# JanSpindler/NRC-HPM-Renderer

Hardware: AMD Instinct MI355X
Metric: Msamples/s + ms/frame at 1080p, 256^3 cloud (NRC path) (higher is better)
Workload: dtype f16 (fp16 MFMA operands, fp32 accumulate; fp32 integrator)

## Files before the change

include/nrc_hpm.h:

```cpp
#ifndef NRC_HPM_H
#define NRC_HPM_H
#include <stddef.h>
#include <stdint.h>

#ifdef __cplusplus
extern "C" {
#endif

#define NRC_OK 0
#define NRC_ERR_INVALID (-1)
#define NRC_ERR_HIP (-2)
#define NRC_ERR_STATE (-3)
#define NRC_ERR_COMM (-4)

const char* nrc_last_error(void);
const char* nrc_version(void);

typedef struct nrc_config {
    char loss_fn[32];
    char optimizer[32];
    float learning_rate;
    float ema_decay;
    uint32_t pos_id;
    uint32_t dir_id;
// ... 130 lines not shown
int nrc_renderer_set_schedule(nrc_renderer_t* r, const nrc_schedule* schedule);
int nrc_renderer_get_schedule(nrc_renderer_t* r, nrc_schedule* current, int* tuning_done);
const char* nrc_renderer_schedule_source(nrc_renderer_t* r);
const char* nrc_renderer_schedule_key(nrc_renderer_t* r);
int nrc_schedule_cache_load(const char* path, int* n_entries);
int nrc_schedule_cache_save(const char* path, int* n_entries);
int nrc_schedule_cache_clear(void);
int nrc_renderer_set_cost_order(nrc_renderer_t* r, int on);
size_t nrc_renderer_tile_order(nrc_renderer_t* r, uint32_t* host_out, size_t capacity);
int nrc_renderer_set_hot_tiles(nrc_renderer_t* r, int on);
int nrc_renderer_hot_tiles(nrc_renderer_t* r, uint32_t* host_out9);
int nrc_renderer_set_full_vertex_images(nrc_renderer_t* r, int on);
size_t nrc_renderer_vertex_image_bytes(nrc_renderer_t* r);
int nrc_renderer_set_stage_events(nrc_renderer_t* r, int on);
int nrc_renderer_count_fetches(nrc_renderer_t* r, int enable, unsigned long long* out);
int nrc_renderer_train_grid(nrc_renderer_t* r, uint32_t out5[5]);

typedef struct nrc_mc_renderer nrc_mc_renderer_t;

int nrc_mc_renderer_create(uint32_t width, uint32_t height, uint32_t path_length, int blend, const nrc_camera* camera,
                           const nrc_scene* scene, const nrc_tile* tile, void* stream, nrc_mc_renderer_t** out);
int nrc_mc_renderer_render(nrc_mc_renderer_t* r);
int nrc_mc_renderer_set_camera(nrc_mc_renderer_t* r, const nrc_camera* camera);
int nrc_mc_renderer_set_blend(nrc_mc_renderer_t* r, int blend);
int nrc_mc_renderer_set_empty_skip(nrc_mc_renderer_t* r, int on);
int nrc_mc_renderer_set_cost_order(nrc_mc_renderer_t* r, int on);
int nrc_mc_renderer_is_blending(nrc_mc_renderer_t* r);
int nrc_mc_renderer_set_scene_params(nrc_mc_renderer_t* r, const nrc_scene* scene);
int nrc_mc_renderer_set_frame_random(nrc_mc_renderer_t* r, const float random4[4]);
const float* nrc_mc_renderer_framebuffer(nrc_mc_renderer_t* r);
int nrc_mc_renderer_export_exr(nrc_mc_renderer_t* r, const char* path);
float nrc_mc_renderer_frame_time_ms(nrc_mc_renderer_t* r);
int nrc_mc_renderer_count_fetches(nrc_mc_renderer_t* r, int enable, unsigned long long* out);
int nrc_mc_renderer_destroy(nrc_mc_renderer_t* r);

int nrc_compare_images(const float* d_ref_rgba, const float* d_own_rgba, uint32_t w, uint32_t h, void* stream,
                       float result5[5]);

int nrc_compare_images_sharded(nrc_cache_t* comm, const float* d_ref_local_rgba, const float* d_own_local_rgba, uint32_t n_local_pixels,
                               void* stream, float result5[5]);

// ... 13 lines not shown
```

nrc-hpm-renderer_amd/api.py:

```python
import ctypes as C
import os

import numpy as np

_HERE = os.path.dirname(os.path.abspath(__file__))
LIB_PATH = os.environ.get("NRC_HPM_LIB") or os.path.join(_HERE, "lib", "libnrc_hpm.so")

NRC_FIX_Q1_TRAIN_Y_DIST = 1
NRC_FIX_Q2_TRAIN_RAY_LEN = 2


class NrcConfig(C.Structure):
    _fields_ = [
        ("loss_fn", C.c_char * 32), ("optimizer", C.c_char * 32),
        ("learning_rate", C.c_float), ("ema_decay", C.c_float),
        ("pos_id", C.c_uint32), ("dir_id", C.c_uint32), ("nn_width", C.c_uint32), ("nn_depth", C.c_uint32),
        ("log2_infer_batch_size", C.c_uint32), ("log2_train_batch_size", C.c_uint32), ("train_batch_count", C.c_uint32),
        ("scene_id", C.c_uint32), ("train_ring_buf_size", C.c_float), ("train_spp", C.c_uint32),
        ("primary_ray_length", C.c_uint32), ("primary_ray_prob", C.c_float), ("train_ray_length", C.c_uint32),
        ("seed", C.c_uint32), ("compat_fix", C.c_uint32), ("hashgrid_log2_size", C.c_uint32),
    ]


class NrcScene(C.Structure):
# ... 29 lines not shown
    "nrc_renderer_set_cost_order", "nrc_renderer_set_schedule", "nrc_renderer_get_schedule", "nrc_renderer_schedule_source", "nrc_renderer_schedule_key",
    "nrc_schedule_cache_load", "nrc_schedule_cache_save", "nrc_schedule_cache_clear", "nrc_renderer_tile_order", "nrc_mc_renderer_set_cost_order", "nrc_renderer_set_hot_tiles", "nrc_renderer_hot_tiles",
    "nrc_cache_get_infer_batch_count", "nrc_cache_get_train_batch_count", "nrc_cache_get_infer_batch_size",
    "nrc_cache_get_train_batch_size", "nrc_cache_infer", "nrc_cache_backward", "nrc_cache_optimizer_step",
    "nrc_cache_grad_ptr", "nrc_cache_param_count", "nrc_cache_loss_ptr", "nrc_cache_set_loss_norm_factor",
    "nrc_comm_unique_id", "nrc_cache_comm_init", "nrc_cache_comm_sparse", "nrc_cache_grid_list_capacity",
    "nrc_cache_set_exchange_dtype", "nrc_cache_get_exchange_dtype",
    "nrc_cache_grid_grad_pack", "nrc_cache_grid_grad_apply",
    "nrc_cache_set_stream", "nrc_cache_set_grad_hook", "nrc_cache_get_params", "nrc_cache_set_params",
    "nrc_cache_get_step", "nrc_cache_set_step", "nrc_cache_param_count_tcnn", "nrc_cache_get_params_tcnn", "nrc_cache_set_params_tcnn",
    "nrc_cache_save_checkpoint", "nrc_cache_load_checkpoint", "nrc_cache_comm_status", "nrc_cache_set_comm_timeout_ms",
    "nrc_renderer_create", "nrc_renderer_render", "nrc_renderer_render_frames", "nrc_renderer_set_stage_events", "nrc_renderer_set_camera", "nrc_renderer_set_blend",
    "nrc_renderer_set_scene_params", "nrc_mc_renderer_set_scene_params",
    "nrc_renderer_set_show_nrc", "nrc_renderer_set_frame_random", "nrc_renderer_framebuffer", "nrc_renderer_framebuffer_on",
    "nrc_renderer_export_exr",
    "nrc_renderer_frame_time_ms", "nrc_renderer_stage_stats", "nrc_renderer_frame_timeline", "nrc_set_wave_priority_raise", "nrc_renderer_destroy", "nrc_renderer_buffer", "nrc_renderer_count_fetches",
    "nrc_renderer_train_grid",
    "nrc_mc_renderer_create", "nrc_mc_renderer_render", "nrc_mc_renderer_set_camera", "nrc_mc_renderer_set_blend",
    "nrc_mc_renderer_set_frame_random", "nrc_mc_renderer_framebuffer", "nrc_mc_renderer_export_exr",
    "nrc_mc_renderer_frame_time_ms", "nrc_mc_renderer_count_fetches", "nrc_mc_renderer_destroy",
    "nrc_compare_images", "nrc_test_math", "nrc_test_rng", "nrc_debug_check_guards", "nrc_image_create", "nrc_image_destroy",
]

_lib = None


def set_wave_priority_raise(on=True):
    _check(load_library().nrc_set_wave_priority_raise(C.c_int(int(bool(on)))))


def build_id():
# ... 581 lines not shown
            return _wrap_device(p, nbytes.value, torch.int32, (nbytes.value // 4,))
        inner = {"primary": 4, "info": 1, "origin": 4, "dir": 4, "infer_input": 5, "infer_output": 3,
                 "train_input": 5, "train_target": 3}[name]
        return _wrap_device(p, nbytes.value, torch.float32, (nbytes.value // (4 * inner), inner))

    def TrainGrid(self):
        o = (C.c_uint32 * 5)()
        _check(self.L.nrc_renderer_train_grid(self.h, o))
        return dict(tw=o[0], th=o[1], x_dist=o[2], y_dist=o[3], ring_size=o[4])

    def CountFetches(self, enable=True):
        v = C.c_ulonglong(0)
        _check(self.L.nrc_renderer_count_fetches(self.h, C.c_int(int(enable)), C.byref(v)))
        return v.value

    def Destroy(self):
        if self.h:
            _check(self.L.nrc_renderer_destroy(self.h))
            self.h = None

    def __del__(self):
        try:
            self.Destroy()
        except Exception:
            pass


class McHpmRenderer:

    def __init__(self, width, height, pathLength, blend, camera, scene, tile=None, stream=None):
# ... 39 lines not shown
        _check(self.L.nrc_mc_renderer_export_exr(self.h, filePath.encode()))

    def GetFrameTimeMS(self):
        return float(self.L.nrc_mc_renderer_frame_time_ms(self.h))

    def GetImage(self):
        import torch
        p = self.L.nrc_mc_renderer_framebuffer(self.h)
        return _wrap_device(p, self.width * self.height * 16, torch.float32, (self.height, self.width, 4))

    def CountFetches(self, enable=True):
        v = C.c_ulonglong(0)
        _check(self.L.nrc_mc_renderer_count_fetches(self.h, C.c_int(int(enable)), C.byref(v)))
        return v.value

    def Destroy(self):
        if self.h:
            _check(self.L.nrc_mc_renderer_destroy(self.h))
            self.h = None

    def __del__(self):
        try:
            self.Destroy()
        except Exception:
            pass


def comm_unique_id():
    buf = (C.c_char * 128)()
    _check(load_library().nrc_comm_unique_id(buf))
# ... 40 lines not shown
```

nrc-hpm-renderer_amd/csrc/nrc_api.hip:

```cpp
#include <algorithm>
#include <array>
#include <chrono>
#include <cmath>
#include <cstdio>
#include <cstdlib>
#include <cstring>
#include <fstream>
#include <map>
#include <memory>
#include <mutex>
#include <random>
#include <string>
#include <thread>
#include <unordered_map>
#include <vector>

#include <dlfcn.h>
#include <rccl/rccl.h>

#include "nrc_integrator.hpp"
#include "nrc_mlp.hpp"
#include "build_id.h"

namespace nrc {
// ... 697 lines not shown
            for (uint32_t y = 0; y < s.ny; y++) {
                const uint8_t* row = s.density + ((size_t)z * s.ny + y) * s.nx;
                const size_t base = ((size_t)(z >> sh) * gy + (y >> sh)) * gx;
                for (uint32_t x = 0; x < s.nx; x++)
                    if (row[x]) {
                        const size_t cidx = base + (x >> sh);
                        bits[cidx >> 5] |= 1u << (cidx & 31);
                    }
            }
        dev_alloc(&d_occ_bits, bits.size() * 4, "d_occ_bits");
        NRC_HIP(hipMemcpy(d_occ_bits, bits.data(), bits.size() * 4, hipMemcpyHostToDevice));
        d.occ_bits = (const uint32_t*)d_occ_bits;
        d.occ_shift = sh; d.occ_gx = gx; d.occ_gy = gy; d.occ_words = (uint32_t)bits.size();
    }

    void build_occupancy(const nrc_scene& s)
    {
        const uint32_t nx = s.nx, ny = s.ny, nz = s.nz;
        const uint32_t gx = (nx + 7) / 8, gy = (ny + 7) / 8, gz = (nz + 7) / 8;
        std::vector<uint8_t> occ((size_t)gx * gy * gz, 0);
        for (uint32_t z = 0; z < nz; z++)
            for (uint32_t y = 0; y < ny; y++) {
                const uint8_t* row = s.density + ((size_t)z * ny + y) * nx;
                const uint32_t cz0 = (z ? z - 1 : 0) >> 3, cz1 = std::min(z + 1, nz - 1) >> 3;
                const uint32_t cy0 = (y ? y - 1 : 0) >> 3, cy1 = std::min(y + 1, ny - 1) >> 3;
                for (uint32_t x = 0; x < nx; x++) {
                    if (row[x] == 0) continue;
                    const uint32_t cx0 = (x ? x - 1 : 0) >> 3, cx1 = std::min(x + 1, nx - 1) >> 3;
                    for (uint32_t cz = cz0; cz <= cz1; cz++)
                        for (uint32_t cy = cy0; cy <= cy1; cy++)
// ... 37 lines not shown
        d.fnx = (float)s.nx; d.fny = (float)s.ny; d.fnz = (float)s.nz;
        float size[3] = {s.size[0], s.size[1], s.size[2]};
        if (size[0] == 0.0f && size[1] == 0.0f && size[2] == 0.0f) {
            const float l = sqrtf((d.fnx * d.fnx + d.fny * d.fny) + d.fnz * d.fnz);
            size[0] = d.fnx / l * 107.5f; size[1] = d.fny / l * 107.5f; size[2] = d.fnz / l * 107.5f;
        }
        for (int k = 0; k < 3; k++) {
            d.size[k] = size[k];
            d.half_size[k] = size[k] * 0.5f;
            d.inv_size[k] = 1.0f / size[k];
        }
        const float tx = 2.0f * size[0], ty = 2.0f * size[1], tz = 2.0f * size[2];
        d.len2size = sqrtf(fmaf(tz, tz, fmaf(ty, ty, tx * tx)));
        build_occupancy(s);
        build_occupancy_bits(s);
        set_params(s);
        d.env = nullptr; d.env_w = d.env_h = 0;
        if (s.env && s.env_w && s.env_h) {
            const size_t eb = (size_t)s.env_w * s.env_h * 16;
            dev_alloc(&d_env, eb, "d_env");
            NRC_HIP(hipMemcpy(d_env, s.env, eb, hipMemcpyHostToDevice));
            d.env = (const float*)d_env; d.env_w = s.env_w; d.env_h = s.env_h;
        }
    }
    void set_params(const nrc_scene& s)
    {
        if (!(s.density_factor > 0.0f)) fail("scene density factor must be positive");
        d.density_factor = s.density_factor;
        d.inv_max_density = 1.0f / s.density_factor;
        d.g = s.g;
// ... 814 lines not shown
    {
        if (frame_index_ > 0)
            NRC_HIP(hipStreamWaitEvent(consumer, ev_comp_done_[(frame_index_ - 1) % (uint64_t)kGenSets], 0));
    }
    void release_frame(hipStream_t consumer)
    {
        if (!ev_consumer_) NRC_HIP(hipEventCreateWithFlags(&ev_consumer_, hipEventDisableTiming));
        NRC_HIP(hipEventRecord(ev_consumer_, consumer));
        consumer_pending_ = true;
    }
    bool is_blending() const { return blend_; }
    void set_full_vertex_images(bool on) { full_vertex_images_ = on; }
    size_t vertex_image_bytes() const { return (full_vertex_images_ ? (size_t)w_ * h_ : (size_t)tg_.tw * tg_.th) * 32; }
    const float* framebuffer_unordered() const { return (const float*)d_out_; }
    const TrainGrid& train_grid() const { return tg_; }
    hipStream_t stream() const { return stream_; }

private:
    void alloc(void** p, size_t bytes)
    {
        dev_alloc(p, bytes, "renderer buffer");
        NRC_HIP(hipMemset(*p, 0, bytes));
        allocs_.push_back(*p);
    }

    void calc_train_subset(uint32_t train_pixel_count)
    {
        const uint32_t sq = (uint32_t)std::sqrt((double)train_pixel_count);
        for (uint32_t factor = sq; factor >= 2; factor--) {
            if (train_pixel_count % factor == 0) {
// ... 326 lines not shown
        timed_ = true;
    }
    void set_cost_order(bool on) { cost_order_ = on; }
    void set_camera(const nrc_camera& c)
    {
        cam_ = to_dev(c);
        nrc_cam_ = c;
        mask_dirty_ = true;
        order_fresh_ = 2;
        blend_index_ = 1;
        NRC_HIP(hipMemsetAsync(d_out_, 0, (size_t)w_ * h_ * 16, stream_));
    }
    void set_scene_params(const nrc_scene& s) { scene_.set_params(s); mask_dirty_ = true; }
    void set_blend(bool b) { blend_ = b; blend_index_ = 1; }
    bool is_blending() const { return blend_; }
    void set_frame_random(const float* r) { std::memcpy(pinned_random_, r, 16); have_pinned_random_ = true; }
    void set_count_fetches(bool on) { count_fetches_ = on; NRC_HIP(hipMemsetAsync(d_fetch_, 0, 8, stream_)); }
    unsigned long long fetches()
    {
        unsigned long long v = 0;
        NRC_HIP(hipMemcpyAsync(&v, d_fetch_, 8, hipMemcpyDeviceToHost, stream_));
        NRC_HIP(hipStreamSynchronize(stream_));
        return v;
    }
    float frame_time_ms()
    {
        if (!timed_) return 0.0f;
        float ms = 0;
        NRC_HIP(hipEventSynchronize(ev_[1]));
        NRC_HIP(hipEventElapsedTime(&ms, ev_[0], ev_[1]));
// ... 548 lines not shown
    NRC_REQUIRE(cam); NRC_REQUIRE(scene); NRC_REQUIRE(out);
    return guarded([&] { *out = new nrc_mc_renderer(w, h, path_length, blend != 0, *cam, *scene, tile, (hipStream_t)stream); });
}
int nrc_mc_renderer_render(nrc_mc_renderer_t* r) { NRC_REQUIRE(r); return guarded([&] { r->impl.render(); }); }
int nrc_mc_renderer_set_camera(nrc_mc_renderer_t* r, const nrc_camera* c) { NRC_REQUIRE(r); NRC_REQUIRE(c); return guarded([&] { r->impl.set_camera(*c); }); }
int nrc_mc_renderer_set_blend(nrc_mc_renderer_t* r, int b) { NRC_REQUIRE(r); r->impl.set_blend(b != 0); return NRC_OK; }
int nrc_mc_renderer_set_frame_random(nrc_mc_renderer_t* r, const float* v) { NRC_REQUIRE(r); NRC_REQUIRE(v); r->impl.set_frame_random(v); return NRC_OK; }
const float* nrc_mc_renderer_framebuffer(nrc_mc_renderer_t* r) { return r ? r->impl.framebuffer() : nullptr; }
int nrc_mc_renderer_export_exr(nrc_mc_renderer_t* r, const char* path) { NRC_REQUIRE(r); NRC_REQUIRE(path); return guarded([&] { r->impl.export_exr(path); }); }
float nrc_mc_renderer_frame_time_ms(nrc_mc_renderer_t* r)
{
    float v = -1.0f;
    if (r) guarded([&] { v = r->impl.frame_time_ms(); });
    return v;
}
int nrc_mc_renderer_count_fetches(nrc_mc_renderer_t* r, int enable, unsigned long long* out)
{
    NRC_REQUIRE(r);
    return guarded([&] { if (out) *out = r->impl.fetches(); r->impl.set_count_fetches(enable != 0); });
}
int nrc_mc_renderer_destroy(nrc_mc_renderer_t* r)
{
    if (!r) return NRC_OK;
    return guarded([&] { delete r; });
}

int nrc_compare_images(const float* d_ref, const float* d_own, uint32_t w, uint32_t h, void* stream, float result5[5])
{
    NRC_REQUIRE(d_ref); NRC_REQUIRE(d_own); NRC_REQUIRE(result5);
    return guarded([&] {
// ... 97 lines not shown
```

nrc-hpm-renderer_amd/csrc/nrc_integrator.hip:

```cpp
#include "nrc_integrator.hpp"

#include <cstdlib>
#include <string>

#include "nrc_math.h"

#ifndef NRC_OCC_ALWAYS
#define NRC_OCC_ALWAYS 0
#endif
#ifndef NRC_CAMERA_WAVES_PER_SIMD
#define NRC_CAMERA_WAVES_PER_SIMD 5
#endif

namespace nrc {
namespace {

struct V3 {
    float x, y, z;
};
__device__ __forceinline__ V3 v3(float x, float y, float z) { return V3{x, y, z}; }
__device__ __forceinline__ V3 add(V3 a, V3 b) { return v3(a.x + b.x, a.y + b.y, a.z + b.z); }
__device__ __forceinline__ V3 sub(V3 a, V3 b) { return v3(a.x - b.x, a.y - b.y, a.z - b.z); }
__device__ __forceinline__ V3 mul(V3 a, float s) { return v3(a.x * s, a.y * s, a.z * s); }
__device__ __forceinline__ V3 neg(V3 a) { return v3(-a.x, -a.y, -a.z); }
// ... 84 lines not shown
        }                                                                                 \
    } while (0)
#define NRC_PROF_LIVE(which, mask)                                                           \
    do {                                                                                     \
        const int n_ = __popcll(mask);                                                       \
        if (n_ > 0 && (threadIdx.x & 63u) == 0u) {                                           \
            const int cls_ = n_ <= 1 ? 0 : n_ <= 2 ? 1 : n_ <= 4 ? 2 : n_ <= 8 ? 3 : n_ <= 16 ? 4 : n_ <= 32 ? 5 : 6; \
            atomicAdd(&g_live_hist[which][cls_], 1ull);                                      \
        }                                                                                    \
    } while (0)
#else
#define NRC_PROF(c, k) do { } while (0)
#define NRC_PROF_LIVE(which, mask) do { } while (0)
#endif

template <bool COUNT>
struct CtxT {
    const DevScene& sc;
    float rng;
    uint32_t fetches;
    __amdgpu_buffer_rsrc_t vol = __builtin_amdgcn_make_buffer_rsrc((void*)sc.density, 0, (int)(sc.nx * sc.ny * sc.nz), 0x00020000);
    const uint32_t* occ = nullptr;
#ifdef NRC_LOOP_PROFILE
    uint32_t useful[8] = {0, 0, 0, 0, 0, 0, 0, 0}, issued[8] = {0, 0, 0, 0, 0, 0, 0, 0};
    uint32_t fee_kind = 1;
#endif
#ifdef NRC_DIAG_CUT_TAIL2
    uint32_t cut2 = 0;
#endif
    __device__ __forceinline__ float rand(float max_val)
    {
        rng = random1(rng);
        return rng * max_val;
    }
    __device__ __forceinline__ void count(uint32_t n)
    {
        if constexpr (COUNT) fetches += n;
    }
};

__device__ __forceinline__ const uint32_t* load_occupancy(const DevScene& sc, uint32_t* s_occ)
{
    fill_log_table();
    if (sc.occ_bits == nullptr) return nullptr;
    for (uint32_t i = threadIdx.x; i < sc.occ_words; i += blockDim.x) s_occ[i] = sc.occ_bits[i];
    __syncthreads();
    return s_occ;
}
__device__ __forceinline__ const uint32_t* load_occupancy_per_wave(const DevScene& sc, uint32_t* s_occ)
{
    fill_log_table();
    if (sc.occ_bits == nullptr) return nullptr;
    const uint4* src = reinterpret_cast<const uint4*>(sc.occ_bits);
    uint4* dst = reinterpret_cast<uint4*>(s_occ);
    for (uint32_t i = threadIdx.x & 63u; i < (sc.occ_words >> 2); i += 64u) dst[i] = src[i];
// ... 81 lines not shown
    const uint32_t ix = (uint32_t)fx, iy = (uint32_t)fy, iz = (uint32_t)fz;
    uint32_t idx = index24(iz, s.ny, iy, s.nx, ix);
    idx = inb ? idx : 0u;
    const uint8_t t = s.density[idx];
    const float d = s.density_factor * ((float)t * (1.0f / 255.0f));
    return inb ? d : 0.0f;
}

struct Addr2 {
    uint32_t i0, i1;
};
struct Fetch2 {
    uint32_t b0, b1;
};
template <class C>
__device__ __forceinline__ Addr2 fetch2_addr(const C& c, V3 dir, V3 start, float t1, float t2, bool first, bool second)
{
    const DevScene& s = c.sc;
    const f2 t = f2{t1, t2};
    const f2 px = fma2(splat(dir.x), t, splat(start.x));
    const f2 py = fma2(splat(dir.y), t, splat(start.y));
    const f2 pz = fma2(splat(dir.z), t, splat(start.z));
    const f2 u = fma2(px, splat(s.inv_size[0]), splat(0.5f));
    const f2 v = fma2(py, splat(s.inv_size[1]), splat(0.5f));
    const f2 w = fma2(pz, splat(s.inv_size[2]), splat(0.5f));
    const f2 fx = u * splat(s.fnx), fy = v * splat(s.fny), fz = w * splat(s.fnz);
    bool in0 = (max(max(nrc_f2u(u.x), nrc_f2u(v.x)), nrc_f2u(w.x)) < 0x3f800000u) & first;
    bool in1 = (max(max(nrc_f2u(u.y), nrc_f2u(v.y)), nrc_f2u(w.y)) < 0x3f800000u) & second;
    const uint32_t x0 = (uint32_t)fx.x, y0 = (uint32_t)fy.x, z0 = (uint32_t)fz.x;
    const uint32_t x1 = (uint32_t)fx.y, y1 = (uint32_t)fy.y, z1 = (uint32_t)fz.y;
    const uint32_t idx0 = index24(z0, s.ny, y0, s.nx, x0);
    const uint32_t idx1 = index24(z1, s.ny, y1, s.nx, x1);
#if !NRC_OCC_ALWAYS
    if (c.occ != nullptr)
#endif
    {
        const uint32_t sh = s.occ_shift;
// ... 621 lines not shown
}

typedef float out_f4 __attribute__((ext_vector_type(4)));
__device__ __forceinline__ void out_store(float4* p, float4 v)
{
    *p = v;
}
__device__ __forceinline__ void out_store(float* p, float v)
{
    *p = v;
}

#ifndef NRC_GEN_WAVES_PER_SIMD
#define NRC_GEN_WAVES_PER_SIMD NRC_CAMERA_WAVES_PER_SIMD
#endif
template <bool COUNT>
__global__ __launch_bounds__(64 * CAMERA_WAVES_PER_BLOCK, NRC_GEN_WAVES_PER_SIMD) void k_gen_rays(DevScene sc, DevCamera cam, DevFrame fr, uint32_t primary_ray_length,
                                                 float primary_ray_prob, float4* __restrict__ primary,
                                                 float* __restrict__ info, float4* __restrict__ origin,
                                                 float4* __restrict__ dirs, float* __restrict__ infer_in,
                                                 unsigned long long* fetch_counter, TrainGrid tg, int full_vertex_images)
{
    camera_wave_priority(fr);
    const unsigned long long t_start = __builtin_amdgcn_s_memtime();
    __shared__ uint32_t s_occ[kOccMaxWords];
    uint32_t lx = 0, y = 0, slot = 0;
    bool inside, hot_wave;
    if (!camera_wave_tile(fr, &lx, &y, &slot, &inside, &hot_wave)) return;
#ifdef NRC_LOOP_PROFILE
    const uint32_t wave_id = blockIdx.x * CAMERA_WAVES_PER_BLOCK + (threadIdx.x >> 6);
    if ((threadIdx.x & 63u) == 0 && wave_id < 65536u) {
        unsigned xcc, hw;
        asm volatile("s_getreg_b32 %0, hwreg(HW_REG_XCC_ID)" : "=s"(xcc));
        asm volatile("s_getreg_b32 %0, hwreg(HW_REG_HW_ID)" : "=s"(hw));
        g_wave_times[4 * wave_id] = wall_clock64();
        g_wave_times[4 * wave_id + 2] = xcc;
        g_wave_times[4 * wave_id + 3] = hw;
    }
#endif
    if (__ballot(inside) == 0ull) return;
    CtxT<COUNT> c{sc, 0.0f, 0u};
    const uint32_t gx = global_x(fr, lx);
    const float u = (float)gx * fr.inv_gw, v = (float)y * fr.inv_gh;
    const float seed_uv = random2(u, v);
    if (fr.hot_next != nullptr) {
        const uint32_t m = nrc_f2u(random2(seed_uv, random4(fr.random_next)) + 1.0f) & 0x007fffffu;
        bool capped = false;
#pragma unroll
        for (uint32_t k = 0; k < kFlightListMax; k++) capped |= (k < fr.flight_n) & (m == fr.flight_list[k]);
        if (__ballot(inside & capped) != 0ull && (threadIdx.x & 63u) == 0u) {
            const uint32_t k = atomicAdd(&fr.hot_next[kHotTilesMax], 1u);
            if (k < kHotTilesMax) fr.hot_next[k] = __builtin_amdgcn_readfirstlane(((y >> 3) << 16) | (lx >> 3));
        }
    }
    if (tile_mask_clear(fr, lx, y)) {
        c.rng = random2(seed_uv, random4(fr.random));
// ... 7 lines not shown
                out_store(&info[pix], 0.0f);
                if (fr.skip_dead_queries == 0u) {
                    float* qo = infer_in + query_index(fr.w, lx, y) * 5u;
#pragma unroll
                    for (int k = 0; k < 5; k++) out_store(&qo[k], 0.0f);
                }
            }
            if (fr.tile_cost != nullptr && !hot_wave && (threadIdx.x & 63u) == 0) store_tile_cost(fr, slot, __builtin_amdgcn_s_memtime() - t_start);
#ifdef NRC_LOOP_PROFILE
            if (inside && full_vertex_images != 0) reinterpret_cast<float*>(origin)[4 * ((size_t)y * fr.w + lx) + 3] = 0.0f;
            if ((threadIdx.x & 63u) == 0 && wave_id < 65536u) g_wave_times[4 * wave_id + 1] = wall_clock64();
#endif
            return;
        }
    }
    c.occ = load_occupancy_per_wave(sc, s_occ);
    V3 ro, rd;
    camera_ray(cam, u, v, &ro, &rd);
    c.rng = random2(seed_uv, random4(fr.random));
    const bool enter = inside;
    V3 entry = ro, ex;
    {
#ifdef NRC_LOOP_PROFILE
        c.fee_kind = 0;
#endif
        find_entry_exit(c, sel(enter, ro, v3(0.0f, 0.0f, 0.0f)), sel(enter, rd, v3(0.0f, 0.0f, 1.0f)), &entry, &ex);
#ifdef NRC_LOOP_PROFILE
        c.fee_kind = 1;
#endif
    }
    const bool entered = enter && !(sky_sdf(sc, entry) > 100000.0f);
// ... 63 lines not shown
        }
    }
#ifdef NRC_LOOP_PROFILE
    if (inside && full_vertex_images != 0) reinterpret_cast<float*>(origin)[4 * ((size_t)y * fr.w + lx) + 3] = (float)c.fetches;
#endif
    if constexpr (COUNT) count_fetches(fetch_counter, c.fetches);
    if (fr.tile_cost != nullptr && !hot_wave && (threadIdx.x & 63u) == 0) store_tile_cost(fr, slot, __builtin_amdgcn_s_memtime() - t_start);
#if defined(NRC_LOOP_PROFILE) && !defined(NRC_NO_LOOP_COUNTERS)
    for (int k = 0; k < 8; k++) { count_fetches(&g_loop_prof[k], c.useful[k]); count_fetches(&g_loop_prof[8 + k], c.issued[k]); }
#endif
#ifdef NRC_LOOP_PROFILE
    if ((threadIdx.x & 63u) == 0 && wave_id < 65536u) g_wave_times[4 * wave_id + 1] = wall_clock64();
#endif
}

template <bool COUNT>
__global__ __launch_bounds__(64 * CAMERA_WAVES_PER_BLOCK, NRC_CAMERA_WAVES_PER_SIMD) void k_mc_render(DevScene sc, DevCamera cam, DevFrame fr, uint32_t path_length,
                                                  float blend_factor, float4* __restrict__ out_rgba,
                                                  float* __restrict__ info, unsigned long long* fetch_counter)
{
    camera_wave_priority(fr);
    const unsigned long long t_start = __builtin_amdgcn_s_memtime();
    __shared__ uint32_t s_occ[kOccMaxWords];
    const uint32_t* occ = load_occupancy(sc, s_occ);
    uint32_t lx = 0, y = 0, slot = 0;
    bool inside, hot_wave;
    if (!camera_wave_tile(fr, &lx, &y, &slot, &inside, &hot_wave)) return;
    CtxT<COUNT> c{sc, 0.0f, 0u};
    c.occ = occ;
    const uint32_t gx = global_x(fr, lx);
    const float u = (float)gx * fr.inv_gw, v = (float)y * fr.inv_gh;
    V3 ro, rd;
    camera_ray(cam, u, v, &ro, &rd);
    init_random(c, u, v, fr.random);
    const bool empty = tile_is_empty(fr, lx, y, inside, c.rng);
    const bool enter = inside & !empty;
    V3 entry = ro, ex;
    if (__ballot(enter) != 0ull) find_entry_exit(c, sel(enter, ro, v3(0.0f, 0.0f, 0.0f)), sel(enter, rd, v3(0.0f, 0.0f, 1.0f)), &entry, &ex);
    const bool entered = enter && !(sky_sdf(sc, entry) > 100000.0f);
    V3 light = v3(0, 0, 0);
    V3 cur = entry, dir = rd;
    float factor = 1.0f;
    bool did_scatter = false, walking = entered;
// ... 166 lines not shown
        push_rank += f;
    }
    if (tid == 0) {
        uint32_t head = ring[0], tail = ring[1];
        if (tg.ring_size > 0) {
            head %= tg.ring_size;
            tail %= tg.ring_size;
        }
        scratch[2 * T] = total;
        scratch[2 * T + 1] = T - total;
        scratch[2 * T + 2] = head;
        scratch[2 * T + 3] = tail;
    }
}

template <int MODE>
__global__ __launch_bounds__(256) void k_prep_train(DevScene sc, DevFrame fr, TrainGrid tg, const float4* __restrict__ origin,
                                                   const float4* __restrict__ dirs, const uint32_t* __restrict__ ring,
                                                   const uint32_t* __restrict__ scratch, float* __restrict__ train_in,
                                                   float* __restrict__ train_target, uint32_t rays_per_wave, float* __restrict__ start)
{
    NRC_RAISE_WAVE_PRIORITY(4);
    __shared__ uint32_t s_occ[kOccMaxWords];
    const uint32_t* occ = load_occupancy(sc, s_occ);
    const uint32_t wave = threadIdx.x >> 6, lane = threadIdx.x & 63u;
    const uint32_t T = tg.tw * tg.th;
    uint32_t tx = blockIdx.x * 16u + (wave & 1u) * 8u + (lane & 7u);
    uint32_t ty = blockIdx.y * 16u + (wave >> 1) * 8u + (lane >> 3);
    bool in_grid = tx < tg.tw && ty < tg.th;
    if (rays_per_wave < 64u) {
        const uint32_t i_lin = ((blockIdx.y * gridDim.x + blockIdx.x) * 4u + wave) * rays_per_wave + lane;
        in_grid = lane < rays_per_wave && i_lin < T;
        tx = in_grid ? i_lin % tg.tw : 0u;
        ty = in_grid ? i_lin / tg.tw : 0u;
    }
    const uint32_t i = in_grid ? ty * tg.tw + tx : 0u;
    CtxT<false> c{sc, 0.0f, 0u};
    c.occ = occ;
    const uint32_t gx = global_x(fr, tx);
    init_random(c, (float)gx * fr.inv_gw, (float)ty * fr.inv_gh, fr.random);
    V3 ro = v3(0, 0, 0);
    V3 rdir = normalize(v3(1.0f, 1.0f, 1.0f));
    if constexpr (MODE == 2) {
        if (in_grid) {
            const float* r = start + 6 * (size_t)i;
            ro = v3(r[0], r[1], r[2]);
            rdir = v3(r[3], r[4], r[5]);
        }
    } else {
        const bool scat = in_grid && scratch[i] != 0u;
        if (scat) {
            const size_t p = (size_t)(ty * tg.y_dist) * fr.w + tx * tg.x_dist;
// ... 275 lines not shown
    float state = random2(random2(u, v), random4(fr));
    out[0] = state;
    for (uint32_t i = 0; i < n; i++) {
        state = random1(state);
        out[1 + i] = state * 1.0f;
    }
}

}

static dim3 pixel_grid(uint32_t w, uint32_t h) { return dim3(ceil_div(w, 16), ceil_div(h, 16)); }
static dim3 wave_tile_grid(uint32_t w, uint32_t h) { return dim3(camera_row_blocks(w) * ceil_div(h, 8)); }

static int g_host_raise_wave_priority = 1;

void launch_gen_rays(const DevScene& sc, const DevCamera& cam, const DevFrame& fr, uint32_t primary_ray_length,
                     float primary_ray_prob, float* primary, float* info, float* origin, float* dir, float* infer_in,
                     unsigned long long* fetch_counter, const TrainGrid& tg, bool full_vertex_images, hipStream_t s)
{
    auto kernel = fetch_counter ? k_gen_rays<true> : k_gen_rays<false>;
#ifdef NRC_LOOP_PROFILE
    kernel = k_gen_rays<true>;
#endif
    dim3 grid = wave_tile_grid(fr.w, fr.h);
    if (fr.hot_tiles != nullptr) grid.x += kHotTilesMax / CAMERA_WAVES_PER_BLOCK;
    DevFrame fa = fr;
    fa.raise_priority = (g_host_raise_wave_priority != 0 && fr.camera_priority_low == 0u) ? 1u : 0u;
    launch_last(kernel, grid, dim3(64 * CAMERA_WAVES_PER_BLOCK), 0u, s, sc, cam, fa,
                primary_ray_length, primary_ray_prob, (float4*)primary, info, (float4*)origin, (float4*)dir, infer_in,
                fetch_counter, tg, full_vertex_images ? 1 : 0);
    NRC_HIP(hipGetLastError());
}

void launch_hot_tiles(const DevFrame& fr, uint32_t* hot, hipStream_t s)
{
    hipLaunchKernelGGL(k_hot_tiles, dim3(4096), dim3(64), 0, s, fr, hot);
    NRC_HIP(hipGetLastError());
// ... 32 lines not shown

void launch_flight_select(const float* table, float lambda, uint32_t* count_and_list, uint32_t* bits, hipStream_t s)
{
    NRC_HIP(hipMemsetAsync(count_and_list, 0, (1 + kFlightListMax) * 4, s));
    hipLaunchKernelGGL(k_flight_select, dim3(kFlightStates / 256u), dim3(256), 0, s, table, lambda, count_and_list, bits);
    NRC_HIP(hipGetLastError());
}

void launch_mc_render(const DevScene& sc, const DevCamera& cam, const DevFrame& fr, uint32_t path_length,
                      float blend_factor, float* out_rgba, float* info, unsigned long long* fetch_counter, hipStream_t s)
{
    dim3 grid = wave_tile_grid(fr.w, fr.h);
    if (fr.hot_tiles != nullptr) grid.x += kHotTilesMax / CAMERA_WAVES_PER_BLOCK;
    DevFrame fa = fr;
    fa.raise_priority = (g_host_raise_wave_priority != 0 && fr.camera_priority_low == 0u) ? 1u : 0u;
    hipLaunchKernelGGL(fetch_counter ? k_mc_render<true> : k_mc_render<false>, grid, dim3(64 * CAMERA_WAVES_PER_BLOCK), 0, s, sc,
                       cam, fa, path_length, blend_factor, (float4*)out_rgba, info, fetch_counter);
    NRC_HIP(hipGetLastError());
}

void launch_prep_train(const DevScene& sc, const DevFrame& fr, const TrainGrid& tg, const float* info, const float* origin,
                       const float* dir, uint32_t* ring, uint32_t* scratch, float* train_in, float* train_target,
                       hipStream_t s, float* start)
{
    const uint32_t T = tg.tw * tg.th;
    hipLaunchKernelGGL(k_train_scan, dim3(1), dim3(1024), 0, s, fr, tg, info, ring, scratch);
    NRC_HIP(hipGetLastError());
    const uint32_t rpw = train_paths_are_long(tg) ? 32u : 64u;
    const dim3 grid = rpw >= 64u ? pixel_grid(tg.tw, tg.th) : dim3(ceil_div(T, 4u * rpw), 1);
    if (start == nullptr)
        hipLaunchKernelGGL(k_prep_train<0>, grid, dim3(256), 0, s, sc, fr, tg, (const float4*)origin, (const float4*)dir, (const uint32_t*)ring,
                           (const uint32_t*)scratch, train_in, train_target, rpw, (float*)nullptr);
    else
        hipLaunchKernelGGL(k_prep_train<1>, pixel_grid(tg.tw, tg.th), dim3(256), 0, s, sc, fr, tg, (const float4*)origin, (const float4*)dir,
                           (const uint32_t*)ring, (const uint32_t*)scratch, train_in, train_target, 64u, start);
    NRC_HIP(hipGetLastError());
    launch_last(k_ring_push, dim3(ceil_div(T, 256)), dim3(256), 0u, s, fr, tg, (const float4*)origin,
                (const float4*)dir, ring, (const uint32_t*)scratch);
    NRC_HIP(hipGetLastError());
}

bool train_paths_are_long(const TrainGrid& tg) { return tg.ray_length * tg.spp >= 4u; }

void launch_train_trace(const DevScene& sc, const DevFrame& fr, const TrainGrid& tg, const float* start, float* train_target, hipStream_t s)
{
    const uint32_t T = tg.tw * tg.th;
    const uint32_t rpw = 32u;
    launch_last(k_prep_train<2>, dim3(ceil_div(T, 4u * rpw), 1), dim3(256), 0u, s, sc, fr, tg, (const float4*)nullptr, (const float4*)nullptr,
                (const uint32_t*)nullptr, (const uint32_t*)nullptr, (float*)nullptr, train_target, rpw, const_cast<float*>(start));
    NRC_HIP(hipGetLastError());
}

void integrator_set_wave_priority_raise(int on)
{
    NRC_HIP(hipMemcpyToSymbol(HIP_SYMBOL(g_raise_wave_priority), &on, sizeof(int)));
    g_host_raise_wave_priority = on;
}

void launch_composite(const DevFrame& fr, uint32_t show_nrc, float blend_factor, const float* primary, const float* info,
                      const float* infer_out, float* out_rgba, hipStream_t s, uint32_t* live_count_reset)
{
    launch_last(k_composite, pixel_grid(fr.w, fr.h), dim3(256), 0u, s, fr, show_nrc, blend_factor,
                (const float4*)primary, info, infer_out, (float4*)out_rgba, live_count_reset);
// ... 92 lines not shown
```

nrc-hpm-renderer_amd/csrc/nrc_integrator.hpp:

```cpp
#pragma once
#include "nrc_common.hpp"

namespace nrc {

struct DevScene {
    const uint8_t* density;
    uint32_t nx, ny, nz;
    float fnx, fny, fnz;
    float size[3], half_size[3], inv_size[3];
    float len2size;
    float density_factor, inv_max_density, g;
    float dir_light_dir[3], dir_light_strength;
    float point_light_pos[3], point_light_strength, point_light_color[3];
    const float* env;
    uint32_t env_w, env_h;
    float env_strength;
    const uint32_t* occ_bits;
    uint32_t occ_shift, occ_gx, occ_gy, occ_words;
};
constexpr uint32_t kOccMaxWords = 2048;

struct DevCamera {
    float m[16];
    float pos[3];
};

struct DevFrame {
    float random[4];
    uint32_t w, h;
    uint32_t x_offset, x_stride;
    uint32_t x_block_log2;
    float inv_gw, inv_gh;
    const uint32_t* tile_mask;
    uint32_t flight_mode, flight_n;
    uint32_t flight_list[8];
// ... 69 lines not shown
```

Before: 8947.

## Specialize volume fetch addressing for power-of-two grids with shift-based indexing

Adds a host-side choice of volume addressing mode (generic, power-of-two, cubic power-of-two with a 32-wide occupancy grid) and templates the gen-rays, MC render and prep-train kernels on it. The specialized path maps positions into voxel coordinates with one fma, checks bounds with integer compares and builds linear and occupancy indices with shifts and bitfield extracts instead of multiplies. The occupancy shared-memory table moves to a single file-scope shared array so the fast path can read it directly. This triples the kernel instantiations, and the fast path indexes the shared table without the occupancy pointer when NRC_OCC_ALWAYS is set, which relies on the table always being loaded.

```diff
diff --git a/include/nrc_hpm.h b/include/nrc_hpm.h
--- a/include/nrc_hpm.h
+++ b/include/nrc_hpm.h
@@ -168,6 +168,7 @@
 size_t nrc_renderer_vertex_image_bytes(nrc_renderer_t* r);
 int nrc_renderer_set_stage_events(nrc_renderer_t* r, int on);
 int nrc_renderer_count_fetches(nrc_renderer_t* r, int enable, unsigned long long* out);
+int nrc_renderer_volume_addressing(nrc_renderer_t* r);
 int nrc_renderer_train_grid(nrc_renderer_t* r, uint32_t out5[5]);
 
 typedef struct nrc_mc_renderer nrc_mc_renderer_t;
@@ -179,6 +180,7 @@
 int nrc_mc_renderer_set_blend(nrc_mc_renderer_t* r, int blend);
 int nrc_mc_renderer_set_empty_skip(nrc_mc_renderer_t* r, int on);
 int nrc_mc_renderer_set_cost_order(nrc_mc_renderer_t* r, int on);
+int nrc_mc_renderer_volume_addressing(nrc_mc_renderer_t* r);
 int nrc_mc_renderer_is_blending(nrc_mc_renderer_t* r);
 int nrc_mc_renderer_set_scene_params(nrc_mc_renderer_t* r, const nrc_scene* scene);
 int nrc_mc_renderer_set_frame_random(nrc_mc_renderer_t* r, const float random4[4]);
diff --git a/nrc-hpm-renderer_amd/api.py b/nrc-hpm-renderer_amd/api.py
--- a/nrc-hpm-renderer_amd/api.py
+++ b/nrc-hpm-renderer_amd/api.py
@@ -67,7 +67,7 @@
     "nrc_renderer_set_scene_params", "nrc_mc_renderer_set_scene_params",
     "nrc_renderer_set_show_nrc", "nrc_renderer_set_frame_random", "nrc_renderer_framebuffer", "nrc_renderer_framebuffer_on",
     "nrc_renderer_export_exr",
-    "nrc_renderer_frame_time_ms", "nrc_renderer_stage_stats", "nrc_renderer_frame_timeline", "nrc_set_wave_priority_raise", "nrc_renderer_destroy", "nrc_renderer_buffer", "nrc_renderer_count_fetches",
+    "nrc_renderer_frame_time_ms", "nrc_renderer_stage_stats", "nrc_renderer_frame_timeline", "nrc_set_wave_priority_raise", "nrc_renderer_destroy", "nrc_renderer_buffer", "nrc_renderer_count_fetches", "nrc_renderer_volume_addressing", "nrc_mc_renderer_volume_addressing",
     "nrc_renderer_train_grid",
     "nrc_mc_renderer_create", "nrc_mc_renderer_render", "nrc_mc_renderer_set_camera", "nrc_mc_renderer_set_blend",
     "nrc_mc_renderer_set_frame_random", "nrc_mc_renderer_framebuffer", "nrc_mc_renderer_export_exr",
@@ -679,6 +679,12 @@
         _check(self.L.nrc_renderer_count_fetches(self.h, C.c_int(int(enable)), C.byref(v)))
         return v.value
 
+    def VolumeAddressing(self):
+        v = self.L.nrc_renderer_volume_addressing(self.h)
+        if v < 0:
+            _check(v)
+        return v
+
     def Destroy(self):
         if self.h:
             _check(self.L.nrc_renderer_destroy(self.h))
@@ -748,6 +754,12 @@
         _check(self.L.nrc_mc_renderer_count_fetches(self.h, C.c_int(int(enable)), C.byref(v)))
         return v.value
 
+    def VolumeAddressing(self):
+        v = self.L.nrc_mc_renderer_volume_addressing(self.h)
+        if v < 0:
+            _check(v)
+        return v
+
     def Destroy(self):
         if self.h:
             _check(self.L.nrc_mc_renderer_destroy(self.h))
diff --git a/nrc-hpm-renderer_amd/csrc/nrc_api.hip b/nrc-hpm-renderer_amd/csrc/nrc_api.hip
--- a/nrc-hpm-renderer_amd/csrc/nrc_api.hip
+++ b/nrc-hpm-renderer_amd/csrc/nrc_api.hip
@@ -735,6 +735,24 @@
         d.occ_shift = sh; d.occ_gx = gx; d.occ_gy = gy; d.occ_words = (uint32_t)bits.size();
     }
 
+    void choose_addressing()
+    {
+        auto pow2 = [](uint32_t n) { return (n & (n - 1u)) == 0u; };
+        auto lg = [](uint32_t n) { uint32_t k = 0; while ((1u << k) < n) k++; return k; };
+        d.addr = kAddrGeneric;
+        for (int k = 0; k < 3; k++) d.lg_n[k] = d.lg_g[k] = 0, d.scale[k] = d.bias[k] = 0.0f;
+        const uint32_t n[3] = {d.nx, d.ny, d.nz};
+        if (!pow2(n[0]) || !pow2(n[1]) || !pow2(n[2])) return;
+        for (int k = 0; k < 3; k++) {
+            d.lg_n[k] = lg(n[k]);
+            d.lg_g[k] = d.lg_n[k] > d.occ_shift ? d.lg_n[k] - d.occ_shift : 0u;
+            d.scale[k] = d.inv_size[k] * (float)n[k];
+            d.bias[k] = 0.5f * (float)n[k];
+        }
+        const bool row = n[0] == n[1] && n[1] == n[2] && d.lg_g[0] == 5u;
+        d.addr = row ? kAddrPow2Row : kAddrPow2;
+    }
+
     void build_occupancy(const nrc_scene& s)
     {
         const uint32_t nx = s.nx, ny = s.ny, nz = s.nz;
@@ -802,6 +820,7 @@
         d.len2size = sqrtf(fmaf(tz, tz, fmaf(ty, ty, tx * tx)));
         build_occupancy(s);
         build_occupancy_bits(s);
+        choose_addressing();
         set_params(s);
         d.env = nullptr; d.env_w = d.env_h = 0;
         if (s.env && s.env_w && s.env_h) {
@@ -1646,6 +1665,7 @@
     size_t vertex_image_bytes() const { return (full_vertex_images_ ? (size_t)w_ * h_ : (size_t)tg_.tw * tg_.th) * 32; }
     const float* framebuffer_unordered() const { return (const float*)d_out_; }
     const TrainGrid& train_grid() const { return tg_; }
+    uint32_t volume_addressing() const { return scene_.d.addr; }
     hipStream_t stream() const { return stream_; }
 
 private:
@@ -2002,6 +2022,7 @@
     void set_scene_params(const nrc_scene& s) { scene_.set_params(s); mask_dirty_ = true; }
     void set_blend(bool b) { blend_ = b; blend_index_ = 1; }
     bool is_blending() const { return blend_; }
+    uint32_t volume_addressing() const { return scene_.d.addr; }
     void set_frame_random(const float* r) { std::memcpy(pinned_random_, r, 16); have_pinned_random_ = true; }
     void set_count_fetches(bool on) { count_fetches_ = on; NRC_HIP(hipMemsetAsync(d_fetch_, 0, 8, stream_)); }
     unsigned long long fetches()
@@ -2580,6 +2601,8 @@
     if (r) guarded([&] { v = r->impl.frame_time_ms(); });
     return v;
 }
+int nrc_renderer_volume_addressing(nrc_renderer_t* r) { return r ? (int)r->impl.volume_addressing() : NRC_ERR_INVALID; }
+int nrc_mc_renderer_volume_addressing(nrc_mc_renderer_t* r) { return r ? (int)r->impl.volume_addressing() : NRC_ERR_INVALID; }
 int nrc_mc_renderer_count_fetches(nrc_mc_renderer_t* r, int enable, unsigned long long* out)
 {
     NRC_REQUIRE(r);
diff --git a/nrc-hpm-renderer_amd/csrc/nrc_integrator.hip b/nrc-hpm-renderer_amd/csrc/nrc_integrator.hip
--- a/nrc-hpm-renderer_amd/csrc/nrc_integrator.hip
+++ b/nrc-hpm-renderer_amd/csrc/nrc_integrator.hip
@@ -122,8 +122,9 @@
 #define NRC_PROF_LIVE(which, mask) do { } while (0)
 #endif
 
-template <bool COUNT>
+template <bool COUNT, uint32_t ADDR = kAddrGeneric>
 struct CtxT {
+    static constexpr uint32_t kAddr = ADDR;
     const DevScene& sc;
     float rng;
     uint32_t fetches;
@@ -147,6 +148,7 @@
     }
 };
 
+__shared__ __attribute__((aligned(16))) uint32_t s_occ_tab[kOccMaxWords];
 __device__ __forceinline__ const uint32_t* load_occupancy(const DevScene& sc, uint32_t* s_occ)
 {
     fill_log_table();
@@ -258,6 +260,50 @@
     uint32_t b0, b1;
 };
 template <class C>
+__device__ __forceinline__ Addr2 fetch2_addr_pow2(const C& c, f2 px, f2 py, f2 pz, bool first, bool second)
+{
+    const DevScene& s = c.sc;
+    constexpr bool row = C::kAddr == kAddrPow2Row;
+    const f2 fx = fma2(px, splat(s.scale[0]), splat(s.bias[0]));
+    const f2 fy = fma2(py, splat(s.scale[1]), splat(row ? s.bias[0] : s.bias[1]));
+    const f2 fz = fma2(pz, splat(s.scale[2]), splat(row ? s.bias[0] : s.bias[2]));
+    bool in0, in1;
+    if constexpr (row) {
+        const uint32_t bn = nrc_f2u(s.fnx);
+        in0 = (max(max(nrc_f2u(fx.x), nrc_f2u(fy.x)), nrc_f2u(fz.x)) < bn) & first;
+        in1 = (max(max(nrc_f2u(fx.y), nrc_f2u(fy.y)), nrc_f2u(fz.y)) < bn) & second;
+    } else {
+        const uint32_t bx = nrc_f2u(s.fnx), by = nrc_f2u(s.fny), bz = nrc_f2u(s.fnz);
+        in0 = nrc_f2u(fx.x) < bx && nrc_f2u(fy.x) < by && nrc_f2u(fz.x) < bz && first;
+        in1 = nrc_f2u(fx.y) < bx && nrc_f2u(fy.y) < by && nrc_f2u(fz.y) < bz && second;
+    }
+    const uint32_t x0 = (uint32_t)fx.x, y0 = (uint32_t)fy.x, z0 = (uint32_t)fz.x;
+    const uint32_t x1 = (uint32_t)fx.y, y1 = (uint32_t)fy.y, z1 = (uint32_t)fz.y;
+    const uint32_t lx = s.lg_n[0], ly = row ? s.lg_n[0] : s.lg_n[1];
+    const uint32_t idx0 = (((z0 << ly) | y0) << lx) | x0;
+    const uint32_t idx1 = (((z1 << ly) | y1) << lx) | x1;
+#if !NRC_OCC_ALWAYS
+    if (c.occ != nullptr)
+#endif
+    {
+        const uint32_t sh = s.occ_shift;
+        if constexpr (row) {
+            const uint32_t w0 = (__builtin_amdgcn_ubfe(z0, sh, 5u) << 5) | __builtin_amdgcn_ubfe(y0, sh, 5u);
+            const uint32_t w1 = (__builtin_amdgcn_ubfe(z1, sh, 5u) << 5) | __builtin_amdgcn_ubfe(y1, sh, 5u);
+            in0 &= __builtin_amdgcn_ubfe(s_occ_tab[w0], x0 >> sh, 1u) != 0u;
+            in1 &= __builtin_amdgcn_ubfe(s_occ_tab[w1], x1 >> sh, 1u) != 0u;
+        } else {
+            const uint32_t gx = s.lg_g[0], gy = s.lg_g[1], gz = s.lg_g[2];
+            const uint32_t c0 = (((__builtin_amdgcn_ubfe(z0, sh, gz) << gy) | __builtin_amdgcn_ubfe(y0, sh, gy)) << gx) | __builtin_amdgcn_ubfe(x0, sh, gx);
+            const uint32_t c1 = (((__builtin_amdgcn_ubfe(z1, sh, gz) << gy) | __builtin_amdgcn_ubfe(y1, sh, gy)) << gx) | __builtin_amdgcn_ubfe(x1, sh, gx);
+            in0 &= __builtin_amdgcn_ubfe(s_occ_tab[c0 >> 5], c0, 1u) != 0u;
+            in1 &= __builtin_amdgcn_ubfe(s_occ_tab[c1 >> 5], c1, 1u) != 0u;
+        }
+    }
+    return Addr2{in0 ? idx0 : 0x80000000u, in1 ? idx1 : 0x80000000u};
+}
+
+template <class C>
 __device__ __forceinline__ Addr2 fetch2_addr(const C& c, V3 dir, V3 start, float t1, float t2, bool first, bool second)
 {
     const DevScene& s = c.sc;
@@ -265,6 +311,7 @@
     const f2 px = fma2(splat(dir.x), t, splat(start.x));
     const f2 py = fma2(splat(dir.y), t, splat(start.y));
     const f2 pz = fma2(splat(dir.z), t, splat(start.z));
+    if constexpr (C::kAddr != kAddrGeneric) return fetch2_addr_pow2(c, px, py, pz, first, second);
     const f2 u = fma2(px, splat(s.inv_size[0]), splat(0.5f));
     const f2 v = fma2(py, splat(s.inv_size[1]), splat(0.5f));
     const f2 w = fma2(pz, splat(s.inv_size[2]), splat(0.5f));
@@ -916,7 +963,7 @@
 #ifndef NRC_GEN_WAVES_PER_SIMD
 #define NRC_GEN_WAVES_PER_SIMD NRC_CAMERA_WAVES_PER_SIMD
 #endif
-template <bool COUNT>
+template <bool COUNT, uint32_t ADDR>
 __global__ __launch_bounds__(64 * CAMERA_WAVES_PER_BLOCK, NRC_GEN_WAVES_PER_SIMD) void k_gen_rays(DevScene sc, DevCamera cam, DevFrame fr, uint32_t primary_ray_length,
                                                  float primary_ray_prob, float4* __restrict__ primary,
                                                  float* __restrict__ info, float4* __restrict__ origin,
@@ -925,7 +972,6 @@
 {
     camera_wave_priority(fr);
     const unsigned long long t_start = __builtin_amdgcn_s_memtime();
-    __shared__ uint32_t s_occ[kOccMaxWords];
     uint32_t lx = 0, y = 0, slot = 0;
     bool inside, hot_wave;
     if (!camera_wave_tile(fr, &lx, &y, &slot, &inside, &hot_wave)) return;
@@ -941,7 +987,7 @@
     }
 #endif
     if (__ballot(inside) == 0ull) return;
-    CtxT<COUNT> c{sc, 0.0f, 0u};
+    CtxT<COUNT, ADDR> c{sc, 0.0f, 0u};
     const uint32_t gx = global_x(fr, lx);
     const float u = (float)gx * fr.inv_gw, v = (float)y * fr.inv_gh;
     const float seed_uv = random2(u, v);
@@ -979,7 +1025,7 @@
             return;
         }
     }
-    c.occ = load_occupancy_per_wave(sc, s_occ);
+    c.occ = load_occupancy_per_wave(sc, s_occ_tab);
     V3 ro, rd;
     camera_ray(cam, u, v, &ro, &rd);
     c.rng = random2(seed_uv, random4(fr.random));
@@ -1073,19 +1119,18 @@
 #endif
 }
 
-template <bool COUNT>
+template <bool COUNT, uint32_t ADDR>
 __global__ __launch_bounds__(64 * CAMERA_WAVES_PER_BLOCK, NRC_CAMERA_WAVES_PER_SIMD) void k_mc_render(DevScene sc, DevCamera cam, DevFrame fr, uint32_t path_length,
                                                   float blend_factor, float4* __restrict__ out_rgba,
                                                   float* __restrict__ info, unsigned long long* fetch_counter)
 {
     camera_wave_priority(fr);
     const unsigned long long t_start = __builtin_amdgcn_s_memtime();
-    __shared__ uint32_t s_occ[kOccMaxWords];
-    const uint32_t* occ = load_occupancy(sc, s_occ);
+    const uint32_t* occ = load_occupancy(sc, s_occ_tab);
     uint32_t lx = 0, y = 0, slot = 0;
     bool inside, hot_wave;
     if (!camera_wave_tile(fr, &lx, &y, &slot, &inside, &hot_wave)) return;
-    CtxT<COUNT> c{sc, 0.0f, 0u};
+    CtxT<COUNT, ADDR> c{sc, 0.0f, 0u};
     c.occ = occ;
     const uint32_t gx = global_x(fr, lx);
     const float u = (float)gx * fr.inv_gw, v = (float)y * fr.inv_gh;
@@ -1282,15 +1327,14 @@
     }
 }
 
-template <int MODE>
+template <int MODE, uint32_t ADDR>
 __global__ __launch_bounds__(256) void k_prep_train(DevScene sc, DevFrame fr, TrainGrid tg, const float4* __restrict__ origin,
                                                    const float4* __restrict__ dirs, const uint32_t* __restrict__ ring,
                                                    const uint32_t* __restrict__ scratch, float* __restrict__ train_in,
                                                    float* __restrict__ train_target, uint32_t rays_per_wave, float* __restrict__ start)
 {
     NRC_RAISE_WAVE_PRIORITY(4);
-    __shared__ uint32_t s_occ[kOccMaxWords];
-    const uint32_t* occ = load_occupancy(sc, s_occ);
+    const uint32_t* occ = load_occupancy(sc, s_occ_tab);
     const uint32_t wave = threadIdx.x >> 6, lane = threadIdx.x & 63u;
     const uint32_t T = tg.tw * tg.th;
     uint32_t tx = blockIdx.x * 16u + (wave & 1u) * 8u + (lane & 7u);
@@ -1303,7 +1347,7 @@
         ty = in_grid ? i_lin / tg.tw : 0u;
     }
     const uint32_t i = in_grid ? ty * tg.tw + tx : 0u;
-    CtxT<false> c{sc, 0.0f, 0u};
+    CtxT<false, ADDR> c{sc, 0.0f, 0u};
     c.occ = occ;
     const uint32_t gx = global_x(fr, tx);
     init_random(c, (float)gx * fr.inv_gw, (float)ty * fr.inv_gh, fr.random);
@@ -1609,13 +1653,16 @@
 
 static int g_host_raise_wave_priority = 1;
 
+#define NRC_BY_ADDR(sc, K, ARG) \
+    ((sc).addr == kAddrPow2Row ? K<ARG, kAddrPow2Row> : (sc).addr == kAddrPow2 ? K<ARG, kAddrPow2> : K<ARG, kAddrGeneric>)
+
 void launch_gen_rays(const DevScene& sc, const DevCamera& cam, const DevFrame& fr, uint32_t primary_ray_length,
                      float primary_ray_prob, float* primary, float* info, float* origin, float* dir, float* infer_in,
                      unsigned long long* fetch_counter, const TrainGrid& tg, bool full_vertex_images, hipStream_t s)
 {
-    auto kernel = fetch_counter ? k_gen_rays<true> : k_gen_rays<false>;
+    auto kernel = fetch_counter ? NRC_BY_ADDR(sc, k_gen_rays, true) : NRC_BY_ADDR(sc, k_gen_rays, false);
 #ifdef NRC_LOOP_PROFILE
-    kernel = k_gen_rays<true>;
+    kernel = NRC_BY_ADDR(sc, k_gen_rays, true);
 #endif
     dim3 grid = wave_tile_grid(fr.w, fr.h);
     if (fr.hot_tiles != nullptr) grid.x += kHotTilesMax / CAMERA_WAVES_PER_BLOCK;
@@ -1678,7 +1725,7 @@
     if (fr.hot_tiles != nullptr) grid.x += kHotTilesMax / CAMERA_WAVES_PER_BLOCK;
     DevFrame fa = fr;
     fa.raise_priority = (g_host_raise_wave_priority != 0 && fr.camera_priority_low == 0u) ? 1u : 0u;
-    hipLaunchKernelGGL(fetch_counter ? k_mc_render<true> : k_mc_render<false>, grid, dim3(64 * CAMERA_WAVES_PER_BLOCK), 0, s, sc,
+    hipLaunchKernelGGL(fetch_counter ? NRC_BY_ADDR(sc, k_mc_render, true) : NRC_BY_ADDR(sc, k_mc_render, false), grid, dim3(64 * CAMERA_WAVES_PER_BLOCK), 0, s, sc,
                        cam, fa, path_length, blend_factor, (float4*)out_rgba, info, fetch_counter);
     NRC_HIP(hipGetLastError());
 }
@@ -1693,10 +1740,10 @@
     const uint32_t rpw = train_paths_are_long(tg) ? 32u : 64u;
     const dim3 grid = rpw >= 64u ? pixel_grid(tg.tw, tg.th) : dim3(ceil_div(T, 4u * rpw), 1);
     if (start == nullptr)
-        hipLaunchKernelGGL(k_prep_train<0>, grid, dim3(256), 0, s, sc, fr, tg, (const float4*)origin, (const float4*)dir, (const uint32_t*)ring,
+        hipLaunchKernelGGL(NRC_BY_ADDR(sc, k_prep_train, 0), grid, dim3(256), 0, s, sc, fr, tg, (const float4*)origin, (const float4*)dir, (const uint32_t*)ring,
                            (const uint32_t*)scratch, train_in, train_target, rpw, (float*)nullptr);
     else
-        hipLaunchKernelGGL(k_prep_train<1>, pixel_grid(tg.tw, tg.th), dim3(256), 0, s, sc, fr, tg, (const float4*)origin, (const float4*)dir,
+        hipLaunchKernelGGL(NRC_BY_ADDR(sc, k_prep_train, 1), pixel_grid(tg.tw, tg.th), dim3(256), 0, s, sc, fr, tg, (const float4*)origin, (const float4*)dir,
                            (const uint32_t*)ring, (const uint32_t*)scratch, train_in, train_target, 64u, start);
     NRC_HIP(hipGetLastError());
     launch_last(k_ring_push, dim3(ceil_div(T, 256)), dim3(256), 0u, s, fr, tg, (const float4*)origin,
@@ -1710,7 +1757,7 @@
 {
     const uint32_t T = tg.tw * tg.th;
     const uint32_t rpw = 32u;
-    launch_last(k_prep_train<2>, dim3(ceil_div(T, 4u * rpw), 1), dim3(256), 0u, s, sc, fr, tg, (const float4*)nullptr, (const float4*)nullptr,
+    launch_last(NRC_BY_ADDR(sc, k_prep_train, 2), dim3(ceil_div(T, 4u * rpw), 1), dim3(256), 0u, s, sc, fr, tg, (const float4*)nullptr, (const float4*)nullptr,
                 (const uint32_t*)nullptr, (const uint32_t*)nullptr, (float*)nullptr, train_target, rpw, const_cast<float*>(start));
     NRC_HIP(hipGetLastError());
 }
diff --git a/nrc-hpm-renderer_amd/csrc/nrc_integrator.hpp b/nrc-hpm-renderer_amd/csrc/nrc_integrator.hpp
--- a/nrc-hpm-renderer_amd/csrc/nrc_integrator.hpp
+++ b/nrc-hpm-renderer_amd/csrc/nrc_integrator.hpp
@@ -17,8 +17,12 @@
     float env_strength;
     const uint32_t* occ_bits;
     uint32_t occ_shift, occ_gx, occ_gy, occ_words;
+    uint32_t addr;
+    uint32_t lg_n[3], lg_g[3];
+    float scale[3], bias[3];
 };
 constexpr uint32_t kOccMaxWords = 2048;
+enum : uint32_t { kAddrGeneric = 0, kAddrPow2 = 1, kAddrPow2Row = 2 };
 
 struct DevCamera {
     float m[16];
```

New measurement: 8983 (median of 6 runs). About the same (+0.4%).
